# mengshanfeng/stencil-2

Hardware: AMD Instinct MI355X
Metric: Jacobi3D Gcells/s (512^3/GPU weak scaling; halo-exchange GB/s in extra) (higher is better)
Workload: dtype fp32

## Files before the change

### csrc/include/stencil/kernels/stencil_ops.hpp

```cpp
#pragma once
#include <algorithm>
#include <cstdint>
#include <vector>

#include "stencil/core/geometry.hpp"
#include "stencil/domain/local_domain.hpp"

namespace stencil {

enum class StencilKind : int {
  Jacobi = 0,
  Astaroth = 1,
};

struct Spheres {
  bool enabled = false;
  Dim3 hot, cold;
  int64_t radius = 0;
  static Spheres jacobi(const Rect3 &cReg) {
    Spheres s;
    s.enabled = true;
    s.hot = Dim3(cReg.lo.x + (cReg.hi.x - cReg.lo.x) / 3, (cReg.lo.y + cReg.hi.y) / 2, (cReg.lo.z + cReg.hi.z) / 2);
    s.cold = Dim3(cReg.lo.x + (cReg.hi.x - cReg.lo.x) * 2 / 3, (cReg.lo.y + cReg.hi.y) / 2, (cReg.lo.z + cReg.hi.z) / 2);
    s.radius = (cReg.hi.x - cReg.lo.x) / 10;
    return s;
  }
};

struct StencilTune {
  int variant = 2;
  static constexpr int kMfma = 8;
  int ty = 2;
  int zchunk = 0;
  int nw = 8;
  int x3sched = 1;
  int x3parts = 0;
  float x3sphw = 0.45f;
  float x2sphw = 0.15f;
  bool x3sphchunk = true;
  int x3left = 3;
  bool x2early = true;
  int x2row = 1;
  int x2sched = 1;
  int x2xfast = 0;
  int x2reserve = 8;
  int reserveCUs = 0;
  bool x2lockstep = true;
  bool zslabRow = true;
  bool xcdRemap = true;
  bool nontemporal = true;
  bool alternateZ = true;
  int wrap = 0;
  uint64_t *publish = nullptr;
  uint64_t *blockClock = nullptr;
  int publishDepth = 0;
};
bool stencil7x2_row_kernel_used(const LocalDomain &dom, int64_t qi, const Rect3 &region, const StencilTune &tune);
int stencil7x2_wrappable_axes(const LocalDomain &dom, int64_t qi, int x2row = 1);

struct ForwardTarget {
  Dim3 dir;
  const LocalDomain *dst;
  Dim3 offset;
};

class HaloForwarder {
public:
  HaloForwarder(const LocalDomain &src, int64_t qi, const std::vector<ForwardTarget> &targets);
  ~HaloForwarder();
  HaloForwarder(const HaloForwarder &) = delete;
  HaloForwarder &operator=(const HaloForwarder &) = delete;
  const int *wm() const { return wm_; }
  const int *wp() const { return wp_; }
  int num_targets() const { return n_; }
  uint32_t mask(int parity) const { return mask_[parity]; }
  int64_t delta(int parity, int k) const { return delta_[parity][k]; }
  bool has_rest() const { return hasRest_; }
  void forward_rest(int parity, hipStream_t stream) const;
  static bool supported(const LocalDomain &dom, int64_t qi);

private:
  int wm_[3] = {0, 0, 0}, wp_[3] = {0, 0, 0};
  int n_ = 0;
  int dev_ = -1;
  uint32_t mask_[2] = {0, 0};
  int64_t delta_[2][27] = {};
  CopyPlan rest_[2];
  bool hasRest_ = false;
};

struct X3PlanInfo {
  int parts = 0, blocks = 0, groups = 0, lockstepGroups = 0, rounds = 0;
// ... 46 lines not shown
      r.rounds = 2;
    }
  }
  return r;
}

inline int64_t slots_less_reserved(int64_t resident, int reserveCUs, int cus) {
  const int64_t perCU = std::max<int64_t>(1, resident / std::max(1, cus));
  return std::max<int64_t>(perCU, resident - perCU * std::min(reserveCUs, cus / 2));
}

enum class X2Form : int { Row = 0, Ragged2, Ragged3, Tail, Col2, Column };
inline bool x2_row_form(X2Form f) { return f <= X2Form::Tail; }
inline bool x2_row_width(int64_t nx) { return nx > 256 && nx <= 832; }
inline X2Form stencil7x2_form(int64_t elemSize, int64_t nx, int64_t x0, int wrap, int x2row, bool publishing,
                              int64_t bufferBytes) {
  if (!x2row) return X2Form::Column;
  const int64_t V = 16 / elemSize, cw = 128 * V;
  const bool onChunk = x0 % V == 0;
  if (elemSize == 4 && (wrap & 1) && onChunk && x2_row_width(nx) && bufferBytes < (int64_t(1) << 32) - 4096) {
    return nx == 512 ? X2Form::Row : nx < 512 ? X2Form::Ragged2 : nx <= 768 ? X2Form::Ragged3 : X2Form::Tail;
  }
  return !publishing && onChunk && nx % cw == 0 ? X2Form::Col2 : X2Form::Column;
}

struct X2SweepSchedule {
  int seg = 1, parts = 0, rounds = 1;
  int64_t blocks = 0;
  int zc = 1, gz = 1;
};
X2SweepSchedule stencil7x2_schedule(X2Form form, int64_t cols, int nz, int64_t resident, int64_t slots,
                                    const StencilTune &tune);
struct X2LaunchInfo {
  X2Form form = X2Form::Column;
  int wrapVariant = 0;
  int64_t cols = 0, slots = 0;
  int seg = 0, parts = 0, rounds = 1;
  int64_t blocks = 0;
  int zchunk = 0, gz = 0;
};
X2LaunchInfo stencil7x2_launch_info(const LocalDomain &dom, int64_t qi, const Rect3 &region, StencilKind kind,
                                    const Spheres &sph, const StencilTune &tune = StencilTune());

struct X3Schedule {
  int seg = 1, parts = 0;
  int64_t blocks = 0;
  int rounds = 1;
};
X3Schedule stencil7x3_schedule(bool xh, int64_t cols, int64_t nz, int64_t slots, const StencilTune &tune,
                               bool publishing);
struct X3LaunchInfo {
  bool supported = false;
  bool xh = false, ragged = false;
  int64_t cols = 0, slots = 0;
  int seg = 0, parts = 0;
  int64_t blocks = 0;
  int rounds = 0;
};
X3LaunchInfo stencil7x3_launch_info(const LocalDomain &dom, int64_t qi, const Rect3 &region, StencilKind kind,
                                    const Spheres &sph, const StencilTune &tune);

int stencil7_wrappable_axes(const LocalDomain &dom, int64_t qi);
bool stencil7_mfma_supported(const LocalDomain &dom, int64_t qi);
void stencil7_mfma_apply(const LocalDomain &dom, int64_t qi, const Rect3 &region, StencilKind kind, const Spheres &sph,
                         hipStream_t stream, const StencilTune &tune = StencilTune());
void stencil7_apply_regions(const LocalDomain &dom, int64_t qi, const std::vector<Rect3> &regions, StencilKind kind,
                            const Spheres &sph, hipStream_t stream, const StencilTune &tune = StencilTune());

struct StarWeights {
  int radius = 1;
  double center = 0;
  double w[3][2][3] = {};
};
bool stencil_star_supported(const LocalDomain &dom, int64_t qi, const StarWeights &w);
void stencil_star_apply(const LocalDomain &dom, int64_t qi, const Rect3 &region, const StarWeights &w,
                        hipStream_t stream, const StencilTune &tune = StencilTune());
struct StarLaunchInfo {
  int path = 0;
  int zchunk = 0;
  int zchunks = 0;
  int64_t blocks = 0;
};
StarLaunchInfo stencil_star_launch_info(const LocalDomain &dom, int64_t qi, const Rect3 &region, const StarWeights &w,
                                        const StencilTune &tune = StencilTune());

struct BoxWeights {
  double w[3][3][3] = {};
};
bool stencil_box_supported(const LocalDomain &dom, int64_t qi);
void stencil_box_apply(const LocalDomain &dom, int64_t qi, const Rect3 &region, const BoxWeights &w,
                       hipStream_t stream, const StencilTune &tune = StencilTune());
struct BoxLaunchInfo {
  int path = 0;
  int zchunk = 0;
  int zchunks = 0;
  int64_t blocks = 0;
};
BoxLaunchInfo stencil_box_launch_info(const LocalDomain &dom, int64_t qi, const Rect3 &region, const BoxWeights &w,
                                      const StencilTune &tune = StencilTune());

struct VarCoefWeights {
  double shift = 0;
  double h[3] = {0, 0, 0};
};
bool stencil_varcoef_supported(const LocalDomain &dom, int64_t qu, int64_t qk);
void stencil_varcoef_apply(const LocalDomain &dom, int64_t qu, int64_t qk, const Rect3 &region, const VarCoefWeights &w,
// ... 27 lines not shown
```

### csrc/python/bindings.cpp

```cpp
#include <pybind11/functional.h>
#include <pybind11/pybind11.h>
#include <pybind11/stl.h>

#include <cstring>

#include <cmath>
#include <limits>
#include <sstream>

#include "stencil/comm/proc_group.hpp"
#include "stencil/comm/ipc_event.hpp"
#include "stencil/comm/rccl_comm.hpp"
#include "stencil/domain/distributed_domain.hpp"
#include "stencil/kernels/copy.hpp"
#include "stencil/kernels/grid_transfer.hpp"
#include "stencil/kernels/stencil_ops.hpp"
#include "stencil/models/stencil_model.hpp"
#include "stencil/rt/build_info.hpp"
#include "stencil/rt/statistics.hpp"
#include "stencil/topo/gpu_topology.hpp"
#include "stencil/topo/partition.hpp"
#include "stencil/topo/placement.hpp"
#include "stencil/topo/qap.hpp"

// ... 1228 lines not shown
                        const std::vector<BoundaryConditions> &bcs) {
          const FillLaunchInfo r = boundary_fill_launch_info(dd.domains().at(di), dd.size(), fill_requests(qs, bcs, true));
          static const char *names[] = {"none", "host", "generic", "fast"};
          py::dict o;
          o["path"] = names[r.path + 1];
          o["boxes"] = r.boxes;
          o["blocks"] = r.blocks;
          o["launches"] = r.launches;
          return o;
        },
        py::arg("dd"), py::arg("domain"), py::arg("qs"), py::arg("bcs"));
  m.def("set_boundary_fill_nontemporal", &set_boundary_fill_nontemporal, py::arg("on"));
  py::class_<X3PlanInfo>(m, "X3PlanInfo")
      .def_readonly("parts", &X3PlanInfo::parts)
      .def_readonly("blocks", &X3PlanInfo::blocks)
      .def_readonly("groups", &X3PlanInfo::groups)
      .def_readonly("lockstep_groups", &X3PlanInfo::lockstepGroups)
      .def_readonly("rounds", &X3PlanInfo::rounds)
      .def_readonly("tabled", &X3PlanInfo::tabled)
      .def_readonly("steps", &X3PlanInfo::steps)
      .def_readonly("zb", &X3PlanInfo::zb)
      .def_readonly("l0", &X3PlanInfo::l0)
      .def_readonly("l1", &X3PlanInfo::l1)
      .def_readonly("odd", &X3PlanInfo::odd)
      .def_readonly("marches", &X3PlanInfo::marches);
  m.def(
      "stencil7x3_plan",
      [](py::handle size, bool jacobi, py::object tune, int slots) {
        return stencil7x3_plan(to_dim3(size), jacobi, tune.is_none() ? StencilTune() : tune.cast<StencilTune>(), slots);
      },
      py::arg("size"), py::arg("jacobi"), py::arg("tune") = py::none(), py::arg("slots") = 256);
  m.def(
      "stencil7x3_schedule",
      [](bool xh, int64_t cols, int64_t nz, int64_t slots, py::object tune, bool publishing) {
        const X3Schedule r = stencil7x3_schedule(xh, cols, nz, slots,
                                                 tune.is_none() ? StencilTune() : tune.cast<StencilTune>(), publishing);
        return py::make_tuple(r.seg, r.parts, r.blocks, r.rounds);
      },
      py::arg("xh"), py::arg("cols"), py::arg("nz"), py::arg("slots"), py::arg("tune") = py::none(),
      py::arg("publishing") = false,
      "launch schedule of a fused-triple sweep (no GPU): (seg, parts, blocks, rounds) for the XH form (xh, columns with "
      "x halos) or the whole-row form over cols (row group, column) pairs of nz planes on `slots` resident blocks; seg "
      "1 = balanced split, 2 = lockstep parts plus second segments, 3 = lockstep rounds (XH form, not publishing)");
  m.def(
      "stencil7x3_launch_info",
      [](DistributedDomain &dd, size_t di, int64_t q, StencilKind kind, bool spheres, const StencilTune &tune) {
        const Spheres s = spheres ? Spheres::jacobi(dd.get_compute_region()) : Spheres();
        const LocalDomain &d = dd.domains().at(di);
        const X3LaunchInfo r = stencil7x3_launch_info(d, q, d.get_compute_region(), kind, s, tune);
        py::dict o;
        o["supported"] = r.supported;
        o["form"] = !r.supported ? "none" : (r.xh ? "xh" : "wrap");
        o["ragged"] = r.ragged;
        o["cols"] = r.cols;
        o["slots"] = r.slots;
        o["seg"] = r.seg;
        o["parts"] = r.parts;
        o["blocks"] = r.blocks;
        o["rounds"] = r.rounds;
        return o;
      },
      py::arg("dd"), py::arg("domain"), py::arg("qi"), py::arg("kind"), py::arg("spheres"), py::arg("tune"));
  m.def(
      "x2_lockstep_schedule",
      [](int64_t slots, int64_t cols, int64_t nz) {
        const X2Schedule r = x2_lockstep_schedule(slots, cols, nz);
        return py::make_tuple(r.parts, r.blocks, r.rounds);
      },
      py::arg("slots"), py::arg("cols"), py::arg("nz"),
      "lockstep schedule of the whole-row / two-chunk-column fused pairs: (z parts per row group, blocks, rounds of "
      "whole columns); (0, 0, 1) = balanced split");
  static const char *x2FormNames[] = {"row", "ragged2", "ragged3", "tail", "col2", "column"};
  m.def(
      "stencil7x2_form",
      [](int64_t elemSize, int64_t nx, int64_t x0, int wrap, int x2row, bool publishing, int64_t bufferBytes) {
        return x2FormNames[int(stencil7x2_form(elemSize, nx, x0, wrap, x2row, publishing, bufferBytes))];
      },
      py::arg("elem_size"), py::arg("nx"), py::arg("x0") = 0, py::arg("wrap") = 1, py::arg("x2row") = 1,
      py::arg("publishing") = false, py::arg("buffer_bytes") = 0,
      "kernel form of a fused-pair sweep (no GPU): \"row\" (512-cell periodic rows), \"ragged2\" / \"ragged3\" (257-511 / "
      "513-768 cells), \"tail\" (769-832), \"col2\" (two-chunk columns), \"column\" (the one-chunk column kernel); x0 = "
      "the region's first x cell counted from the first interior cell");
  m.def(
      "stencil7x2_schedule",
      [](const std::string &form, int64_t cols, int nz, int64_t resident, int64_t slots, py::object tune) {
        int f = 0;
        while (f < 6 && form != x2FormNames[f]) ++f;
        STENCIL_REQUIRE(f < 6, "fused-pair form " << form);
        const X2SweepSchedule r = stencil7x2_schedule(X2Form(f), cols, nz, resident, slots,
                                                      tune.is_none() ? StencilTune() : tune.cast<StencilTune>());
        py::dict o;
        o["seg"] = r.seg;
        o["parts"] = r.parts;
        o["rounds"] = r.rounds;
        o["blocks"] = r.blocks;
        o["zchunk"] = r.zc;
        o["gz"] = r.gz;
        return o;
      },
      py::arg("form"), py::arg("cols"), py::arg("nz"), py::arg("resident"), py::arg("slots"),
      py::arg("tune") = py::none(),
      "block schedule of a fused-pair sweep (no GPU): seg 0 = fixed z chunks (zchunk planes, gz per column), 1 = "
      "balanced split, 2 = lockstep parts plus second segments, 3 = lockstep rounds");
  m.def("slots_less_reserved", &slots_less_reserved, py::arg("resident"), py::arg("reserve_cus"), py::arg("cus"),
        "resident blocks a launch may fill when it leaves reserve_cus of the device's cus CUs to another stream");
  m.def(
      "stencil7x2_launch_info",
      [](DistributedDomain &dd, size_t di, int64_t q, const Rect3 &region, StencilKind kind, bool spheres,
         const StencilTune &tune) {
        const Spheres s = spheres ? Spheres::jacobi(dd.get_compute_region()) : Spheres();
        const X2LaunchInfo r = stencil7x2_launch_info(dd.domains().at(di), q, region, kind, s, tune);
        py::dict o;
        o["form"] = x2FormNames[int(r.form)];
        o["wrap_variant"] = r.wrapVariant;
        o["cols"] = r.cols;
        o["slots"] = r.slots;
        o["seg"] = r.seg;
        o["parts"] = r.parts;
        o["rounds"] = r.rounds;
        o["blocks"] = r.blocks;
        o["zchunk"] = r.zchunk;
        o["gz"] = r.gz;
        return o;
      },
      py::arg("dd"), py::arg("domain"), py::arg("qi"), py::arg("region"), py::arg("kind"), py::arg("spheres"),
      py::arg("tune"));
  m.def("jacobi_spheres", [](const Rect3 &cReg) {
    Spheres s = Spheres::jacobi(cReg);
    return py::make_tuple(s.hot, s.cold, s.radius);
  });

  py::class_<StencilTune>(m, "StencilTune")
      .def(py::init<>())
      .def_readwrite("variant", &StencilTune::variant)
      .def_readwrite("ty", &StencilTune::ty)
      .def_readwrite("zchunk", &StencilTune::zchunk)
      .def_readwrite("xcd_remap", &StencilTune::xcdRemap)
      .def_readwrite("nontemporal", &StencilTune::nontemporal)
      .def_readwrite("alternate_z", &StencilTune::alternateZ)
      .def_readwrite("nw", &StencilTune::nw)
      .def_readwrite("x3sched", &StencilTune::x3sched)
      .def_readwrite("x2early", &StencilTune::x2early)
      .def_readwrite("x3parts", &StencilTune::x3parts)
      .def_readwrite("x3sphw", &StencilTune::x3sphw)
      .def_readwrite("x3sphchunk", &StencilTune::x3sphchunk)
      .def_readwrite("x3left", &StencilTune::x3left)
      .def_readwrite("x2sphw", &StencilTune::x2sphw)
      .def_property(
          "block_clock", [](const StencilTune &t) { return reinterpret_cast<uintptr_t>(t.blockClock); },
          [](StencilTune &t, uintptr_t p) { t.blockClock = reinterpret_cast<uint64_t *>(p); })
      .def_readwrite("x2row", &StencilTune::x2row)
      .def_readwrite("x2sched", &StencilTune::x2sched)
      .def_readwrite("x2reserve", &StencilTune::x2reserve)
      .def_readwrite("wrap", &StencilTune::wrap)
      .def_readwrite("x2lockstep", &StencilTune::x2lockstep)
      .def_readwrite("zslab_row", &StencilTune::zslabRow)
      .def_readwrite("x2xfast", &StencilTune::x2xfast);
  py::class_<StencilModelConfig>(m, "StencilModelConfig")
      .def(py::init<>())
      .def_readwrite("size", &StencilModelConfig::size)
      .def_readwrite("kind", &StencilModelConfig::kind)
      .def_readwrite("radius", &StencilModelConfig::radius)
      .def_readwrite("all_directions", &StencilModelConfig::allDirections)
      .def_readwrite("quantities", &StencilModelConfig::quantities)
      .def_readwrite("fp64", &StencilModelConfig::fp64)
      .def_readwrite("methods", &StencilModelConfig::methods)
      .def_readwrite("placement", &StencilModelConfig::placement)
      .def_readwrite("axis_cost", &StencilModelConfig::axisCost)
      .def_readwrite("partition", &StencilModelConfig::partition)
      .def_readwrite("gpus", &StencilModelConfig::gpus)
      .def_readwrite("overlap", &StencilModelConfig::overlap)
      .def_readwrite("auto_overlap", &StencilModelConfig::autoOverlap)
      .def_readwrite("use_graph", &StencilModelConfig::useGraph)
      .def_readwrite("forward", &StencilModelConfig::forward)
      .def_readwrite("temporal", &StencilModelConfig::temporal)
      .def_readwrite("wrap_self", &StencilModelConfig::wrapSelf)
      .def_readwrite("x_halo_align", &StencilModelConfig::xHaloAlign)
      .def_readwrite("shared_halo_line", &StencilModelConfig::sharedHaloLine)
      .def_readwrite("interior_align", &StencilModelConfig::interiorAlign)
      .def_readwrite("row_pad_lines", &StencilModelConfig::rowPadLines)
      .def_readwrite("wrap_axes_mask", &StencilModelConfig::wrapAxesMask)
      .def_readwrite("local_interior", &StencilModelConfig::localInterior)
      .def_readwrite("overlap_mode", &StencilModelConfig::overlapMode)
      .def_readwrite("transport", &StencilModelConfig::transport)
      .def_readwrite("self_test", &StencilModelConfig::selfTest)
      .def_property(
          "backend", [](const StencilModelConfig &c) { return c.backend; },
          [](StencilModelConfig &c, Backend b) {
            c.backend = b;
            c.setBackend = true;
          })
      .def_readwrite("tune", &StencilModelConfig::tune)
      .def_readwrite("astaroth_period", &StencilModelConfig::astarothPeriod);
  py::class_<StencilModel, std::shared_ptr<StencilModel>>(m, "StencilModel")
      .def(py::init([](const StencilModelConfig &c, std::shared_ptr<comm::ProcGroup> pg) {
             py::gil_scoped_release r;
             return std::make_shared<StencilModel>(c, pg);
           }),
// ... 34 lines not shown
```

### csrc/src/kernels/stencil7x3.hip

```cpp
#include <hip/hip_runtime.h>

#include <algorithm>
#include <map>
#include <mutex>
#include <utility>
#include <vector>
#include <cmath>
#include <cstring>

#include "stencil/kernels/stencil_ops.hpp"
#include "stencil/rt/hip_check.hpp"
#include "stencil_common.hpp"
#include "stencil_wave.hpp"

namespace stencil {

struct X3Seg {
  uint32_t s, e, s2, e2;
  bool odd;
  bool odd2;
};
template <typename T>
__host__ __device__ __forceinline__ X3Seg x3_segments(const StencilArgs<T> &a, const ZPartBounds &B, uint32_t lb,
                                                      uint32_t nb, uint32_t ncols, uint32_t gy, uint32_t nzt) {
// ... 407 lines not shown
            for (int h = 0; h < H; ++h) {
              U1b[h] = U1c[h];
              U1c[h] = U1a[h];
              U2b[h] = U2c[h];
              U2c[h] = U2a[h];
            }
            if constexpr (EDGE) {
              U1Eb = U1Ec;
              U1Ec = U1Ea;
            }
            ++t;
            return true;
          };
          using I0 = std::integral_constant<int, 0>;
          using I1 = std::integral_constant<int, 1>;
          using I2 = std::integral_constant<int, 2>;
          using I3 = std::integral_constant<int, 3>;
          using L1 = std::integral_constant<int, (RM < 1 ? RM : 1)>;
          using L2 = std::integral_constant<int, (RM < 2 ? RM : 2)>;
          using LR = std::integral_constant<int, RM>;
          step(I0{}, L1{});
          step(I1{}, L1{});
          step(I2{}, L2{});
          step(I3{}, L2{});
          while (step(I0{}, LR{}) && step(I1{}, LR{}) && step(I2{}, LR{}) && step(I3{}, LR{})) {
          }
        };
        if (down)
          march(std::true_type{});
        else
          march(std::false_type{});
      }
    }
  };
  const unsigned long long clk0 = a.clk ? wall_clock64() : 0;
  const int role = (w >= 3 && w < NW - 3) ? 3 : ((w >= 2 && w < NW - 2) ? 2 : ((w >= 1 && w < NW - 1) ? 1 : 0));
  if (role == 3)
    body(std::integral_constant<int, 3>{});
  else if (role == 2)
    body(std::integral_constant<int, 2>{});
  else if (role == 1)
    body(std::integral_constant<int, 1>{});
  else
    body(std::integral_constant<int, 4>{});
  if (a.clk) {
    __syncthreads();
    if (lane == 0 && w == 0) {
      a.clk[2 * lb] = clk0;
      a.clk[2 * lb + 1] = wall_clock64();
    }
  }
}

template <int KIND, bool PUB, bool NT>
__global__ __launch_bounds__(64 * 12, 3) __attribute__((amdgpu_waves_per_eu(3, 3))) void
stencil7x3_wrap_kernel(StencilArgs<float> a, ZPartBounds zbounds) {
  constexpr int NW = 12;
  using T = float;
  using NV = nf4;
  constexpr int V = 4, H = 2;
  constexpr int CS = 64 * V;
  constexpr int LS = V;
  constexpr int YO = NW - 6;
  constexpr int NC = 4;
  __shared__ NV cs[2][NW][H][64];
  __shared__ NV us[2][NW][H][64];
  __shared__ NV vs[2][NW][H][64];

  const uint32_t nb = gridDim.x;
  const uint32_t lb = a.remap ? xcd_remap(blockIdx.x, nb) : blockIdx.x;
  const int lane = threadIdx.x;
  const int w = __builtin_amdgcn_readfirstlane(int(threadIdx.y));
  const uint32_t nzt = uint32_t(a.hiz - a.loz);
  const X3Seg sg = x3_segments(a, zbounds, lb, nb, uint32_t(a.gy), uint32_t(a.gy), nzt);
  const bool lane0 = lane == 0, lane63 = lane == 63;
  const int wA = w > 0 ? w - 1 : 0, wB = w < NW - 1 ? w + 1 : NW - 1;
  const int xb = a.lox + lane * LS;
  const int zwn = a.wn[2], zwlo = a.wlo[2], zwhi = a.wlo[2] + a.wn[2];
  const __amdgpu_buffer_rsrc_t srcRsrc =
      __builtin_amdgcn_make_buffer_rsrc(const_cast<float *>(a.src), 0, -1, 0x00020000);
  auto zcl = [&](int zz) {
    zz += zz < zwlo ? zwn : 0;
    zz -= zz >= zwhi ? zwn : 0;
    return zz < 0 ? 0 : (zz > a.rawZm1 ? a.rawZm1 : zz);
  };
  auto body = [&](auto roleTag) {
    constexpr int R = decltype(roleTag)::value;
    bool odd = sg.odd;
    const bool pubOrder = PUB;
    for (int pp = 0; pp < 2; ++pp) {
      const int pass = pubOrder ? 1 - pp : pp;
      uint32_t s = pass == 0 ? sg.s : sg.s2;
      const uint32_t e = pass == 0 ? sg.e : sg.e2;
      if (pass == 1 && !pubOrder) odd = sg.odd2;
      while (s < e) {
        const uint32_t by = s / nzt;
        const int zo = int(s - by * nzt);
        const int nzs = int(min(nzt - uint32_t(zo), e - s));
        s += uint32_t(nzs);
        const int zs = a.loz + zo;
        const int ze = zs + nzs;
        bool down = pass == 0 && sg.odd;
        if (!pubOrder) {
          down = odd != (a.flip != 0);
          odd = !odd;
        }
        const int yblk = a.loy + YO * int(by);
        const int y = yblk - 3 + w;
        if (yblk >= a.hiy) continue;
        const bool outRow = R == 3 && y < a.hiy;
        int yw = y < a.wlo[1] ? y + a.wn[1] : (y >= a.wlo[1] + a.wn[1] ? y - a.wn[1] : y);
        yw = yw < 0 ? 0 : (yw > a.rawYm1 ? a.rawYm1 : yw);
        const uint32_t rowoff = uint32_t((yw * int64_t(a.px) + xb) * int64_t(sizeof(T)));
        const uint32_t outoff = uint32_t((y * int64_t(a.px) + xb) * int64_t(sizeof(T)));

        const int yh = a.r1sq - (y - a.hy) * (y - a.hy), yc = a.r1sq - (y - a.cy) * (y - a.cy);
        struct RowSph {
          int Dh, Dc;
          bool hit;
        };
        auto row_sph = [&](int P) -> RowSph {
          RowSph r{0, 0, false};
          if (KIND == 0) {
            r.Dh = yh - (P - a.hz) * (P - a.hz);
            r.Dc = yc - (P - a.cz) * (P - a.cz);
            r.hit = max(r.Dh, r.Dc) > 0;
          }
          return r;
        };
        auto sphere_row = [&](const RowSph &rs, NV(&o)[H]) {
          if (KIND == 0 && rs.hit) {
            const int Dh = rs.Dh, Dc = rs.Dc;
#pragma unroll
            for (int h = 0; h < H; ++h)
#pragma unroll
              for (int k = 0; k < V; ++k) {
                const int x = xb + h * CS + k;
                const bool hot = (x - a.hx) * (x - a.hx) < Dh;
                const bool cold = (x - a.cx) * (x - a.cx) < Dc;
                o[h][k] = hot ? T(1) : (cold ? T(0) : o[h][k]);
              }
          }
        };
        auto row_update = [&](const NV(&cm)[H], const NV(&up)[H], const NV(&dn)[H], const NV(&zp)[H], const NV(&zm)[H],
                              NV(&o)[H]) -> T {
          static_assert(H == 2, "two chunks per lane");
          const T r30 = rot_prev(cm[0][V - 1]), r31 = rot_prev(cm[1][V - 1]);
          const T l00 = rot_next(cm[0][0]), l01 = rot_next(cm[1][0]);
          NV s6[H];
#pragma unroll
          for (int h = 0; h < H; ++h) {
            const T left = h == 0 ? (lane0 ? r31 : r30) : (lane0 ? r30 : r31);
            const T right = h == 0 ? (lane63 ? l01 : l00) : (lane63 ? l00 : l01);
            NV vpx, vmx;
#pragma unroll
            for (int k = 0; k < V; ++k) {
              vpx[k] = k < V - 1 ? cm[h][k + 1] : right;
              vmx[k] = k > 0 ? cm[h][k - 1] : left;
            }
            s6[h] = sum6v<T, KIND>(vpx, vmx, dn[h], up[h], zp[h], zm[h]);
          }
          float m = 1.0f;
#pragma unroll
          for (int h = 0; h < H; ++h) o[h] = div6v_fast<NV, V>(s6[h], m);
          if (__builtin_expect(m < 0x1p-100f, 0)) {
#pragma unroll
            for (int h = 0; h < H; ++h) div6v_fix<NV, V>(s6[h], o[h]);
          }
          return T(1);
        };

        auto march = [&](auto downTag) {
          constexpr bool DOWN = decltype(downTag)::value;
          constexpr int dz = DOWN ? -1 : 1;
          const int z0 = DOWN ? ze - 1 : zs;
          NV C[NC][H];
          NV U1a[H], U1b[H], U1c[H];
          NV U2a[H], U2b[H], U2c[H];
          auto load_row = [&](int zz, int k) {
            const uint32_t po = uint32_t(zcl(zz)) * uint32_t(a.pxy) * uint32_t(sizeof(T));
#pragma unroll
            for (int h = 0; h < H; ++h)
              C[k][h] = __builtin_bit_cast(
                  NV, __builtin_amdgcn_raw_buffer_load_b128(srcRsrc, rowoff + uint32_t(h * CS * int(sizeof(T))), po, 0));
          };
          {
            const int zw = z0 - 3 * dz;
#pragma unroll
            for (int k = 0; k < NC - 1; ++k) load_row(zw + k * dz, k);
#pragma unroll
// ... 44 lines not shown
                sphere_row(row_sph(z), o);
              }
            };
            levels();
            if constexpr (LV >= 3) {
              char *dp = outRow ? reinterpret_cast<char *>(a.dst + int64_t(z) * a.pxy) + outoff
                                : a.sink + lane * LS * int(sizeof(T));
#pragma unroll
              for (int h = 0; h < H; ++h) {
                NV *q = reinterpret_cast<NV *>(dp + h * CS * int(sizeof(T)));
                if constexpr (NT)
                  __builtin_nontemporal_store(o[h], q);
                else
                  *q = o[h];
              }
            }
            const int nbuf = buf ^ 1;
            if constexpr (LV < 1)
#pragma unroll
              for (int h = 0; h < H; ++h) cs[nbuf][w][h][lane] = C[s2][h];
            const bool pubStep = PUB && t >= 0 && (z < a.pubLo || z >= a.pubHi);
            if (pubStep) asm volatile("s_waitcnt vmcnt(0)" ::: "memory");
            __syncthreads();
            if (pubStep && lane == 0 && w == 0) {
              __builtin_amdgcn_fence(__ATOMIC_RELEASE, "");
              const unsigned long long cells =
                  (unsigned long long)(min(YO, a.hiy - yblk)) * (unsigned long long)(a.hix - a.lox);
              __hip_atomic_fetch_add(a.pub, cells, __ATOMIC_RELAXED, __HIP_MEMORY_SCOPE_SYSTEM);
            }
#pragma unroll
            for (int h = 0; h < H; ++h) {
              U1b[h] = U1c[h];
              U1c[h] = U1a[h];
              U2b[h] = U2c[h];
              U2c[h] = U2a[h];
            }
            ++t;
            return true;
          };
          using I0 = std::integral_constant<int, 0>;
          using I1 = std::integral_constant<int, 1>;
          using I2 = std::integral_constant<int, 2>;
          using I3 = std::integral_constant<int, 3>;
          using L1 = std::integral_constant<int, (R < 1 ? R : 1)>;
          using L2 = std::integral_constant<int, (R < 2 ? R : 2)>;
          using LR = std::integral_constant<int, R>;
          step(I0{}, L1{});
          step(I1{}, L1{});
          step(I2{}, L2{});
          step(I3{}, L2{});
          while (step(I0{}, LR{}) && step(I1{}, LR{}) && step(I2{}, LR{}) && step(I3{}, LR{})) {
          }
        };
        if (down)
          march(std::true_type{});
        else
          march(std::false_type{});
      }
    }
  };
  const unsigned long long clk0 = a.clk ? wall_clock64() : 0;
  const int role = (w >= 3 && w < NW - 3) ? 3 : ((w >= 2 && w < NW - 2) ? 2 : ((w >= 1 && w < NW - 1) ? 1 : 0));
  if (role == 3)
    body(std::integral_constant<int, 3>{});
  else if (role == 2)
    body(std::integral_constant<int, 2>{});
  else if (role == 1)
    body(std::integral_constant<int, 1>{});
  else
    body(std::integral_constant<int, 0>{});
  if (a.clk) {
    __syncthreads();
    if (lane == 0 && w == 0) {
      a.clk[2 * lb] = clk0;
      a.clk[2 * lb + 1] = wall_clock64();
    }
  }
}

template <typename T, int KIND> static const void *x3_wrap_kernel_ptr(bool nt) {
  if constexpr (std::is_same<T, float>::value)
    return nt ? (const void *)stencil7x3_wrap_kernel<KIND, false, true>
              : (const void *)stencil7x3_wrap_kernel<KIND, false, false>;
  else
    return nullptr;
}
template <typename T, int KIND> using X3XhKernel = void (*)(StencilArgs<T>, ZPartBounds);
template <typename T, int KIND, bool BIG, bool PUB> static X3XhKernel<T, KIND> x3_xh_kernel_ptr(bool rag) {
  return rag ? stencil7x3_xh_kernel<T, KIND, BIG, PUB, true> : stencil7x3_xh_kernel<T, KIND, BIG, PUB, false>;
}
template <typename T, int KIND> static X3XhKernel<T, KIND> x3_xh_kernel_ptr(bool big, bool pub, bool rag) {
  return big ? (pub ? x3_xh_kernel_ptr<T, KIND, true, true>(rag) : x3_xh_kernel_ptr<T, KIND, true, false>(rag))
             : (pub ? x3_xh_kernel_ptr<T, KIND, false, true>(rag) : x3_xh_kernel_ptr<T, KIND, false, false>(rag));
}

static std::map<int, char *> gX3Sinks;
static std::mutex gX3SinkMu;
static char *x3_sink(int dev, bool create) {
  std::lock_guard<std::mutex> lk(gX3SinkMu);
  char *&p = gX3Sinks[dev];
  if (!p && create) {
    int cur = 0;
    HIP_CHECK(hipGetDevice(&cur));
    HIP_CHECK(hipSetDevice(dev));
    HIP_CHECK(hipMalloc(reinterpret_cast<void **>(&p), 4096));
    HIP_CHECK(hipSetDevice(cur));
  }
  return p;
}

int64_t stencil7x3_column_cells(int64_t elemSize) { return 2 * 64 * (16 / elemSize); }

bool stencil7x3_supported(const LocalDomain &dom, int64_t qi, const Rect3 &region, const StencilTune &tune) {
  if (dom.backend() != Backend::Device) return false;
  const int64_t es = dom.elem_size(qi);
  const bool f32 = dom.dtype(qi) == DType::F32 || (dom.dtype(qi) == DType::Bytes && es == 4);
  const bool f64 = dom.dtype(qi) == DType::F64 || (dom.dtype(qi) == DType::Bytes && es == 8);
  if (!f32 && !f64) return false;
  const Radius &rad = dom.radius();
  const Dim3 n = dom.size();
  const int wrapm = tune.wrap & 7;
  if (wrapm & 1) {
    if (!f32 || n.x != 512 || !(stencil7x2_wrappable_axes(dom, qi, 1) & 1)) return false;
  } else {
    const int64_t cw = stencil7x3_column_cells(es);
    if (rad.x(-1) < 3 || rad.x(1) < 3 || n.x < 3 || n.x % cw > cw - 3) return false;
  }
  if (!(wrapm & 2) && (rad.y(-1) < 3 || rad.y(1) < 3)) return false;
  if (!(wrapm & 4) && (rad.z(-1) < 3 || rad.z(1) < 3)) return false;
  for (int i = 0; i < 27; ++i) {
    const Dim3 d = dir_from_index(i);
    const int nzc = (d.x != 0) + (d.y != 0) + (d.z != 0);
    const bool halo = !((d.x != 0 && (wrapm & 1)) || (d.y != 0 && (wrapm & 2)) || (d.z != 0 && (wrapm & 4)));
    if (nzc >= 2 && halo && rad.dir(d) < 1) return false;
  }
  const Rect3 cr = dom.get_compute_region();
// ... 63 lines not shown
static X3Plan x3_plan(const StencilArgs<T> &a, bool jac, int64_t cols, int64_t slots, uint32_t blocks,
                      const StencilTune &tune) {
  constexpr int NW = 12, YO = NW - 6;
  constexpr double kUnsync = 1.2;
  const int64_t nz = a.hiz - a.loz;
  const float w = jac ? tune.x3sphw : 0.f;
  auto plan = [&](int P, int64_t nbP, ZPartBounds &b) -> double {
    b = ZPartBounds{};
    const int64_t cm = nbP / P;
    if (jac) sphere_part_bounds(b, a, std::min<int64_t>(cm, a.gy), P, NW, YO, 3, w);
    const int mode = tune.x3left;
    ZPartBounds bg = b, bl = b;
    const double tg = mode == 1 || mode == 3
                          ? balance_leftover(bg, a, nbP, cm, P, cols, a.gy, NW, YO, 3, w, 4, mode == 3 ? kUnsync : 1.0)
                          : -1;
    const double tl = mode == 2 || mode == 3 ? lockstep_leftover(bl, a, nbP, cm, P, cols, a.gy, NW, YO, 3, w, 4, 16) : -1;
    if (tl >= 0 && (tg < 0 || tl <= tg)) {
      b = bl;
      return tl;
    }
    if (tg >= 0) {
      b = bg;
      return tg;
    }
    const std::vector<double> mc = lockstep_part_costs(b, a, cm, P, a.gy, NW, YO, 3, w, 4);
    const double left = cols > cm ? double((cols - cm) * nz) * kUnsync / double(nbP) + 4 : 0;
    return *std::max_element(mc.begin(), mc.end()) + left;
  };
  X3Plan pl{a.zparts, blocks, ZPartBounds{}, 0};
  if (tune.x3sched == 1 && tune.x3parts <= 0 && tune.x3left != 0) {
    double best = -1;
    const bool sph = jac && a.r1sq > 0 && w > 0;
    for (int P = 2; P <= (sph ? kZPartMaxParts : 8); ++P) {
      const int64_t cm = std::min<int64_t>(cols, slots / P);
      if (cm < 1 || nz / P < 16) continue;
      ZPartBounds b;
      const double t = plan(P, P * cm, b);
      if (best < 0 || t < best - 1e-9) {
        best = t;
        pl = X3Plan{P, uint32_t(P * cm), b, t};
      }
    }
  } else {
    pl.steps = plan(a.zparts, int64_t(blocks), pl.b);
  }
  return pl;
}

template <typename T> struct X3Launch {
  StencilArgs<T> a;
  ZPartBounds zb;
  uint32_t blocks;
  bool big, rag;
  int64_t cols, slots;
};
template <typename T, int KIND, bool XH>
static X3Launch<T> x3_prepare(const LocalDomain &dom, int64_t qi, const Rect3 &region, const Spheres &sph,
                              const StencilTune &tune) {
  constexpr int NW = 12, YO = NW - 6;
  X3Launch<T> L{};
  StencilArgs<T> &a = L.a;
  a = make_args<T>(dom, qi, region, KIND == 0 ? StencilKind::Jacobi : StencilKind::Astaroth, sph);
  a.flip = tune.alternateZ ? (dom.parity() & 1) : 0;
  a.nt = tune.nontemporal ? 1 : 0;
  a.wrapm = tune.wrap & 7;
  if (!(a.wrapm & 2)) a.wn[1] = 0;
  if (!(a.wrapm & 4)) a.wn[2] = 0;
  a.x0 = a.lox;
  a.remap = tune.xcdRemap ? 1 : 0;
  a.sphchunk = tune.x3sphchunk ? 1 : 0;
  a.sphr = int(sph.radius);
  const int nx = a.hix - a.lox, ny = a.hiy - a.loy, nz = a.hiz - a.loz;
  const int cw = int(stencil7x3_column_cells(int64_t(sizeof(T))));
  a.gx = XH ? (nx + cw - 1) / cw : 1;
  a.xr = XH ? nx - (a.gx - 1) * cw : nx;
  const bool rag = XH && a.xr < cw;
  a.gy = (ny + YO - 1) / YO;
  const bool big = dom.buffer_bytes(qi) >= (int64_t(1) << 32) - 4096;
  const void *kern =
      XH ? (const void *)x3_xh_kernel_ptr<T, KIND>(big, false, rag) : x3_wrap_kernel_ptr<T, KIND>(a.nt != 0);
  const int64_t cols = int64_t(a.gx) * a.gy;
  const int64_t resident = resident_blocks(kern, 64 * NW, 1);
  const int64_t slots = launch_slots(resident, tune.reserveCUs, dom.gpu());
  if (tune.publish) {
    a.pub = reinterpret_cast<unsigned long long *>(tune.publish);
    a.pubLo = a.loz + tune.publishDepth;
    a.pubHi = a.hiz - tune.publishDepth;
    a.flip = 0;
  }
  const X3Schedule ls = stencil7x3_schedule(XH, cols, nz, slots, tune, tune.publish != nullptr);
  a.seg = ls.seg;
  uint32_t blocks = uint32_t(ls.blocks);
  if (ls.seg != 1) {
    a.zparts = ls.parts;
    a.zrounds = ls.rounds;
  }
  ZPartBounds &zb = L.zb;
  if (a.seg == 2) {
    static std::map<std::vector<int64_t>, X3Plan> cache;
    static std::mutex mu;
    int32_t wbits = 0;
    std::memcpy(&wbits, &tune.x3sphw, sizeof(wbits));
    const std::vector<int64_t> key{KIND, a.loy,  a.hiy, a.loz, a.hiz,          a.hy,        a.cy,
                                   a.hz, a.cz,   a.r1sq, int64_t(blocks), a.zparts, cols, a.gy,
                                   wbits, tune.x3left, tune.x3sched, tune.x3parts, slots};
    std::lock_guard<std::mutex> lk(mu);
    auto it = cache.find(key);
    if (it == cache.end()) it = cache.emplace(key, x3_plan(a, KIND == 0, cols, slots, blocks, tune)).first;
    a.zparts = it->second.P;
    blocks = it->second.blocks;
    zb = it->second.b;
  }
  a.sink = x3_sink(dom.gpu(), false);
  a.clk = reinterpret_cast<unsigned long long *>(tune.blockClock);
  L.blocks = blocks;
  L.big = big;
  L.rag = rag;
  L.cols = cols;
  L.slots = slots;
  return L;
}

template <typename T, int KIND, bool XH>
static void apply_x3_t(const LocalDomain &dom, int64_t qi, const Rect3 &region, const Spheres &sph, hipStream_t stream,
                       const StencilTune &tune) {
  constexpr int NW = 12;
  const X3Launch<T> L = x3_prepare<T, KIND, XH>(dom, qi, region, sph, tune);
  const StencilArgs<T> &a = L.a;
  const ZPartBounds &zb = L.zb;
  const uint32_t blocks = L.blocks;
  dom.set_device();
  STENCIL_REQUIRE(a.sink, "stencil7x3: no store sink on device " << dom.gpu() << " (stencil7x3_supported first)");
  if constexpr (XH || !std::is_same<T, float>::value) {
    const X3XhKernel<T, KIND> k = x3_xh_kernel_ptr<T, KIND>(L.big, a.pub != nullptr, L.rag);
    hipLaunchKernelGGL(k, dim3(blocks), dim3(64, NW), 0, stream, a, zb);
  } else {
    if (a.pub)
      hipLaunchKernelGGL((stencil7x3_wrap_kernel<KIND, true, false>), dim3(blocks), dim3(64, NW), 0, stream, a, zb);
    else if (a.nt)
      hipLaunchKernelGGL((stencil7x3_wrap_kernel<KIND, false, true>), dim3(blocks), dim3(64, NW), 0, stream, a, zb);
    else
      hipLaunchKernelGGL((stencil7x3_wrap_kernel<KIND, false, false>), dim3(blocks), dim3(64, NW), 0, stream, a, zb);
  }
  HIP_CHECK(hipGetLastError());
}

static std::vector<int> x3_marches(const StencilArgs<float> &a, const ZPartBounds &zb, uint32_t nb) {
  constexpr int YO = 6;
  std::vector<int> out;
  const uint32_t nzt = uint32_t(a.hiz - a.loz);
  for (uint32_t lb = 0; lb < nb; ++lb) {
    const X3Seg sg = x3_segments(a, zb, lb, nb, uint32_t(a.gy), uint32_t(a.gy), nzt);
    bool odd = sg.odd;
    for (int pass = 0; pass < 2; ++pass) {
      uint32_t s = pass == 0 ? sg.s : sg.s2;
      const uint32_t e = pass == 0 ? sg.e : sg.e2;
      if (pass == 1) odd = sg.odd2;
      while (s < e) {
        const uint32_t by = s / nzt;
        const int zo = int(s - by * nzt);
        const int nzs = int(std::min(nzt - uint32_t(zo), e - s));
        s += uint32_t(nzs);
        const bool down = odd != (a.flip != 0);
        odd = !odd;
        if (a.loy + YO * int(by) >= a.hiy) continue;
        out.insert(out.end(), {int(lb), int(by), a.loz + zo, nzs, int(down)});
      }
    }
  }
  return out;
}

X3PlanInfo stencil7x3_plan(const Dim3 &size, bool jacobi, const StencilTune &tune, int slots) {
  constexpr int YO = 6;
  StencilArgs<float> a{};
  a.hix = int(size.x);
  a.hiy = int(size.y);
  a.hiz = int(size.z);
  if (jacobi) {
    const Spheres s = Spheres::jacobi(Rect3(Dim3(0, 0, 0), size));
    a.hx = int(s.hot.x);
    a.hy = int(s.hot.y);
    a.hz = int(s.hot.z);
    a.cx = int(s.cold.x);
    a.cy = int(s.cold.y);
    a.cz = int(s.cold.z);
    a.r1sq = int((s.radius + 1) * (s.radius + 1));
  }
  a.gx = 1;
  a.gy = int((size.y + YO - 1) / YO);
  const int64_t cols = a.gy, nz = size.z;
  X3PlanInfo r;
  r.groups = int(cols);
  const X3Schedule ls = stencil7x3_schedule(false, cols, nz, slots, tune, tune.publish != nullptr);
  r.parts = ls.parts;
  r.blocks = ls.seg == 1 ? 0 : int(ls.blocks);
  r.rounds = ls.rounds;
  a.seg = ls.seg;
  if (ls.seg != 2) {
    r.marches = x3_marches(a, ZPartBounds{}, uint32_t(ls.blocks));
    return r;
  }
  a.zparts = ls.parts;
  const X3Plan pl = x3_plan(a, jacobi, cols, slots, uint32_t(ls.blocks), tune);
  a.zparts = pl.P;
  r.marches = x3_marches(a, pl.b, pl.blocks);
  r.parts = pl.P;
  r.blocks = int(pl.blocks);
  r.lockstepGroups = int(pl.blocks) / pl.P;
  r.steps = pl.steps;
  r.tabled = pl.b.lon != 0;
  if (pl.b.on)
    for (int g = 0; g < std::min<int>(r.lockstepGroups, kZPartMaxCols); ++g)
      for (int q = 0; q + 1 < pl.P; ++q) r.zb.push_back(pl.b.zb[g][q]);
  if (r.tabled)
    for (uint32_t lb = 0; lb < pl.blocks; ++lb) {
      r.l0.push_back(pl.b.l0[lb]);
      r.l1.push_back(pl.b.l1[lb]);
      r.odd.push_back(int((pl.b.ldir[lb / 32] >> (lb % 32)) & 1));
    }
  return r;
}

bool stencil7x3_apply(const LocalDomain &dom, int64_t qi, const Rect3 &region, StencilKind kind, const Spheres &sph,
                      hipStream_t stream, const StencilTune &tune) {
  if (!stencil7x3_supported(dom, qi, region, tune)) return false;
  const bool jac = kind == StencilKind::Jacobi, xh = !(tune.wrap & 1);
  if (dom.elem_size(qi) == 8) {
    jac ? apply_x3_t<double, 0, true>(dom, qi, region, sph, stream, tune)
        : apply_x3_t<double, 1, true>(dom, qi, region, sph, stream, tune);
  } else if (xh) {
    jac ? apply_x3_t<float, 0, true>(dom, qi, region, sph, stream, tune)
        : apply_x3_t<float, 1, true>(dom, qi, region, sph, stream, tune);
  } else {
    jac ? apply_x3_t<float, 0, false>(dom, qi, region, sph, stream, tune)
        : apply_x3_t<float, 1, false>(dom, qi, region, sph, stream, tune);
  }
  return true;
}

template <typename T, int KIND, bool XH>
static X3LaunchInfo x3_launch_info_t(const LocalDomain &dom, int64_t qi, const Rect3 &region, const Spheres &sph,
                                     const StencilTune &tune) {
  const X3Launch<T> L = x3_prepare<T, KIND, XH>(dom, qi, region, sph, tune);
  X3LaunchInfo r;
  r.supported = true;
  r.xh = XH;
  r.ragged = L.rag;
  r.cols = L.cols;
  r.slots = L.slots;
  r.seg = L.a.seg;
  r.parts = L.a.seg == 1 ? 0 : L.a.zparts;
  r.blocks = int64_t(L.blocks);
  r.rounds = L.a.seg == 3 ? L.a.zrounds : 1;
  return r;
}

X3LaunchInfo stencil7x3_launch_info(const LocalDomain &dom, int64_t qi, const Rect3 &region, StencilKind kind,
                                    const Spheres &sph, const StencilTune &tune) {
  if (!stencil7x3_supported(dom, qi, region, tune)) return X3LaunchInfo();
  const bool jac = kind == StencilKind::Jacobi, xh = !(tune.wrap & 1);
  if (dom.elem_size(qi) == 8)
    return jac ? x3_launch_info_t<double, 0, true>(dom, qi, region, sph, tune)
               : x3_launch_info_t<double, 1, true>(dom, qi, region, sph, tune);
  if (xh)
    return jac ? x3_launch_info_t<float, 0, true>(dom, qi, region, sph, tune)
               : x3_launch_info_t<float, 1, true>(dom, qi, region, sph, tune);
  return jac ? x3_launch_info_t<float, 0, false>(dom, qi, region, sph, tune)
             : x3_launch_info_t<float, 1, false>(dom, qi, region, sph, tune);
}

}
```

Before: 1942.

## Stage fused-triple wrap march rows via buffer-load-to-LDS DMA ring

Adds a DMA variant of the wrap-form fused triple stencil kernel. Input z-rows are loaded directly into an LDS ring with buffer_load_lds, and intermediate sweep levels are exchanged through LDS, with explicit vmcnt/lgkmcnt waits and barriers per step. The aim is to remove register staging of global loads and overlap prefetch of rows several planes ahead with compute. It adds a sizeable shared-memory array that may reduce residency, and it is enabled by a new x3dma tune flag that defaults on but only applies to the non-publishing wrap form.

New measurement: 1856. 4.4% lower.

```diff
diff --git a/csrc/include/stencil/kernels/stencil_ops.hpp b/csrc/include/stencil/kernels/stencil_ops.hpp
--- a/csrc/include/stencil/kernels/stencil_ops.hpp
+++ b/csrc/include/stencil/kernels/stencil_ops.hpp
@@ -38,6 +38,7 @@
   float x3sphw = 0.45f;
   float x2sphw = 0.15f;
   bool x3sphchunk = true;
+  bool x3dma = true;
   int x3left = 3;
   bool x2early = true;
   int x2row = 1;
@@ -190,6 +191,7 @@
 struct X3LaunchInfo {
   bool supported = false;
   bool xh = false, ragged = false;
+  bool dma = false;
   int64_t cols = 0, slots = 0;
   int seg = 0, parts = 0;
   int64_t blocks = 0;
diff --git a/csrc/python/bindings.cpp b/csrc/python/bindings.cpp
--- a/csrc/python/bindings.cpp
+++ b/csrc/python/bindings.cpp
@@ -1304,6 +1304,7 @@
         o["supported"] = r.supported;
         o["form"] = !r.supported ? "none" : (r.xh ? "xh" : "wrap");
         o["ragged"] = r.ragged;
+        o["dma"] = r.dma;
         o["cols"] = r.cols;
         o["slots"] = r.slots;
         o["seg"] = r.seg;
@@ -1396,6 +1397,7 @@
       .def_readwrite("x3parts", &StencilTune::x3parts)
       .def_readwrite("x3sphw", &StencilTune::x3sphw)
       .def_readwrite("x3sphchunk", &StencilTune::x3sphchunk)
+      .def_readwrite("x3dma", &StencilTune::x3dma)
       .def_readwrite("x3left", &StencilTune::x3left)
       .def_readwrite("x2sphw", &StencilTune::x2sphw)
       .def_property(
diff --git a/csrc/src/kernels/stencil7x3.hip b/csrc/src/kernels/stencil7x3.hip
--- a/csrc/src/kernels/stencil7x3.hip
+++ b/csrc/src/kernels/stencil7x3.hip
@@ -483,9 +483,10 @@
   }
 }
 
-template <int KIND, bool PUB, bool NT>
+template <int KIND, bool PUB, bool NT, bool DMA = false>
 __global__ __launch_bounds__(64 * 12, 3) __attribute__((amdgpu_waves_per_eu(3, 3))) void
 stencil7x3_wrap_kernel(StencilArgs<float> a, ZPartBounds zbounds) {
+  static_assert(!(PUB && DMA), "the publishing instances keep the register-staged march");
   constexpr int NW = 12;
   using T = float;
   using NV = nf4;
@@ -497,6 +498,8 @@
   __shared__ NV cs[2][NW][H][64];
   __shared__ NV us[2][NW][H][64];
   __shared__ NV vs[2][NW][H][64];
+  constexpr int XU1 = 3 * NW, XU2 = XU1 + 2 * (NW - 2), XROWS = XU2 + 2 * (NW - 4);
+  __shared__ NV xl[XROWS * H * 64];
 
   const uint32_t nb = gridDim.x;
   const uint32_t lb = a.remap ? xcd_remap(blockIdx.x, nb) : blockIdx.x;
@@ -562,11 +565,13 @@
         auto sphere_row = [&](const RowSph &rs, NV(&o)[H]) {
           if (KIND == 0 && rs.hit) {
             const int Dh = rs.Dh, Dc = rs.Dc;
+            int xo = xb;
+            if constexpr (DMA) asm volatile("" : "+v"(xo));
 #pragma unroll
             for (int h = 0; h < H; ++h)
 #pragma unroll
               for (int k = 0; k < V; ++k) {
-                const int x = xb + h * CS + k;
+                const int x = xo + h * CS + k;
                 const bool hot = (x - a.hx) * (x - a.hx) < Dh;
                 const bool cold = (x - a.cx) * (x - a.cx) < Dc;
                 o[h][k] = hot ? T(1) : (cold ? T(0) : o[h][k]);
@@ -717,10 +722,157 @@
           while (step(I0{}, LR{}) && step(I1{}, LR{}) && step(I2{}, LR{}) && step(I3{}, LR{})) {
           }
         };
-        if (down)
-          march(std::true_type{});
-        else
-          march(std::false_type{});
+
+        auto march_dma = [&](auto downTag) {
+          constexpr bool DOWN = decltype(downTag)::value;
+          constexpr int dz = DOWN ? -1 : 1;
+          const int z0 = DOWN ? ze - 1 : zs;
+          NV W[3][H];
+          NV NA[H], NB[H];
+          NV U1a[H], U1b[H], U1c[H];
+          NV U2a[H], U2b[H], U2c[H];
+          typedef __attribute__((address_space(3))) NV LNV;
+          auto rowbase = [&](int row) -> uint32_t {
+            uint32_t b = uint32_t(reinterpret_cast<uintptr_t>(&xl[row * H * 64 + lane]));
+            asm("" : "+v"(b));
+            return b;
+          };
+          auto u1row = [&](int r) { return XU1 + min(max(r, 1), NW - 2) - 1; };
+          auto u2row = [&](int r) { return XU2 + min(max(r, 2), NW - 3) - 2; };
+          const uint32_t rW = rowbase(w), rA = rowbase(wA), rB = rowbase(wB);
+          const uint32_t uW = rowbase(u1row(w)), uA = rowbase(u1row(wA)), uB = rowbase(u1row(wB));
+          const uint32_t vW = rowbase(u2row(w)), vA = rowbase(u2row(wA)), vB = rowbase(u2row(wB));
+          auto at = [&](uint32_t base, int off) -> LNV & { return *reinterpret_cast<LNV *>(base + uint32_t(off)); };
+          auto ring = [&](uint32_t base, int slot, int h) -> LNV & { return at(base, (slot * NW * H + h) * 1024); };
+          auto u1s = [&](uint32_t base, int b, int h) -> LNV & { return at(base, (b * (NW - 2) * H + h) * 1024); };
+          auto u2s = [&](uint32_t base, int b, int h) -> LNV & { return at(base, (b * (NW - 4) * H + h) * 1024); };
+          auto dma_row = [&](int zz, int slot) {
+            const uint32_t po = uint32_t(zcl(zz)) * uint32_t(a.pxy) * uint32_t(sizeof(T));
+#pragma unroll
+            for (int h = 0; h < H; ++h)
+              __builtin_amdgcn_raw_ptr_buffer_load_lds(
+                  srcRsrc, (__attribute__((address_space(3))) void *)&xl[((slot * NW + w) * H + h) * 64], 16,
+                  rowoff + uint32_t(h * CS * int(sizeof(T))), po, 0, 0);
+          };
+          {
+            dma_row(z0 - 3 * dz, 0);
+            dma_row(z0 - 2 * dz, 1);
+            dma_row(z0 - dz, 2);
+            asm volatile("s_waitcnt vmcnt(0)" ::: "memory");
+            __builtin_amdgcn_s_barrier();
+#pragma unroll
+            for (int h = 0; h < H; ++h) {
+              W[0][h] = ring(rW, 0, h);
+              W[1][h] = W[2][h] = NA[h] = NB[h] = W[0][h];
+              U1a[h] = U1b[h] = U1c[h] = U2a[h] = U2b[h] = U2c[h] = W[0][h];
+            }
+            asm volatile("s_waitcnt lgkmcnt(0)" ::: "memory");
+          }
+          int t = -5;
+          auto step = [&](auto phase, auto lvTag, auto psTag) -> bool {
+            constexpr int k = decltype(phase)::value;
+            constexpr int LV = decltype(lvTag)::value;
+            constexpr bool PS = decltype(psTag)::value;
+            constexpr int s0 = (k + 1) % 3, s1 = (k + 2) % 3, s2 = k % 3, sn = (k + 2) % 3;
+            constexpr int buf = k & 1;
+            if (t >= nzs) return false;
+            const int z = z0 + t * dz;
+            dma_row(z + 5 * dz, sn);
+            __builtin_amdgcn_sched_barrier(0);
+            NV o[H];
+            if constexpr (R >= 1) {
+              NV A2[H], B2[H], A3[H], B3[H];
+#pragma unroll
+              for (int h = 0; h < H; ++h) W[s2][h] = ring(rW, s2, h);
+              if constexpr (LV >= 1) {
+                (void)row_update(W[s1], NA, NB, DOWN ? W[s0] : W[s2], DOWN ? W[s2] : W[s0], U1a);
+                sphere_row(row_sph(z + 2 * dz), U1a);
+#pragma unroll
+                for (int h = 0; h < H; ++h) u1s(uW, buf ^ 1, h) = U1a[h];
+              }
+#pragma unroll
+              for (int h = 0; h < H; ++h) {
+                NA[h] = ring(rA, s2, h);
+                NB[h] = ring(rB, s2, h);
+              }
+              if constexpr (LV >= 2) {
+#pragma unroll
+                for (int h = 0; h < H; ++h) {
+                  A2[h] = u1s(uA, buf, h);
+                  B2[h] = u1s(uB, buf, h);
+                }
+                (void)row_update(U1c, A2, B2, DOWN ? U1b : U1a, DOWN ? U1a : U1b, U2a);
+                sphere_row(row_sph(z + dz), U2a);
+#pragma unroll
+                for (int h = 0; h < H; ++h) u2s(vW, buf ^ 1, h) = U2a[h];
+              }
+              if constexpr (LV >= 3) {
+#pragma unroll
+                for (int h = 0; h < H; ++h) {
+                  A3[h] = u2s(vA, buf, h);
+                  B3[h] = u2s(vB, buf, h);
+                }
+                (void)row_update(U2c, A3, B3, DOWN ? U2b : U2a, DOWN ? U2a : U2b, o);
+                sphere_row(row_sph(z), o);
+                char *dp = outRow ? reinterpret_cast<char *>(a.dst + int64_t(z) * a.pxy) + outoff
+                                  : a.sink + lane * LS * int(sizeof(T));
+#pragma unroll
+                for (int h = 0; h < H; ++h) {
+                  NV *q = reinterpret_cast<NV *>(dp + h * CS * int(sizeof(T)));
+                  if constexpr (NT)
+                    __builtin_nontemporal_store(o[h], q);
+                  else
+                    *q = o[h];
+                }
+              }
+            }
+            constexpr int N = 2 + (LV >= 3 ? 2 : 0) + (PS ? 2 : 0);
+            asm volatile("s_waitcnt vmcnt(%0)\n\ts_waitcnt lgkmcnt(0)" ::"n"(N) : "memory");
+            __builtin_amdgcn_s_barrier();
+#pragma unroll
+            for (int h = 0; h < H; ++h) {
+              U1b[h] = U1c[h];
+              U1c[h] = U1a[h];
+              U2b[h] = U2c[h];
+              U2c[h] = U2a[h];
+            }
+            ++t;
+            return true;
+          };
+          using I0 = std::integral_constant<int, 0>;
+          using I1 = std::integral_constant<int, 1>;
+          using I2 = std::integral_constant<int, 2>;
+          using I3 = std::integral_constant<int, 3>;
+          using I4 = std::integral_constant<int, 4>;
+          using I5 = std::integral_constant<int, 5>;
+          using L0 = std::integral_constant<int, 0>;
+          using L1 = std::integral_constant<int, (R < 1 ? R : 1)>;
+          using L2 = std::integral_constant<int, (R < 2 ? R : 2)>;
+          using LR = std::integral_constant<int, R>;
+          using PN = std::false_type;
+          using PY = std::integral_constant<bool, R == 3>;
+          step(I1{}, L0{}, PN{});
+          step(I2{}, L1{}, PN{});
+          step(I3{}, L1{}, PN{});
+          step(I4{}, L2{}, PN{});
+          step(I5{}, L2{}, PN{});
+          step(I0{}, LR{}, PN{});
+          while (step(I1{}, LR{}, PY{}) && step(I2{}, LR{}, PY{}) && step(I3{}, LR{}, PY{}) && step(I4{}, LR{}, PY{}) &&
+                 step(I5{}, LR{}, PY{}) && step(I0{}, LR{}, PY{})) {
+          }
+          asm volatile("s_waitcnt vmcnt(0)" ::: "memory");
+        };
+        if constexpr (DMA) {
+          if (down)
+            march_dma(std::true_type{});
+          else
+            march_dma(std::false_type{});
+        } else {
+          if (down)
+            march(std::true_type{});
+          else
+            march(std::false_type{});
+        }
       }
     }
   };
@@ -743,10 +895,15 @@
   }
 }
 
-template <typename T, int KIND> static const void *x3_wrap_kernel_ptr(bool nt) {
+using X3WrapKernel = void (*)(StencilArgs<float>, ZPartBounds);
+template <int KIND> static X3WrapKernel x3_wrap_kernel(bool pub, bool nt, bool dma) {
+  if (pub) return stencil7x3_wrap_kernel<KIND, true, false>;
+  if (dma) return nt ? stencil7x3_wrap_kernel<KIND, false, true, true> : stencil7x3_wrap_kernel<KIND, false, false, true>;
+  return nt ? stencil7x3_wrap_kernel<KIND, false, true> : stencil7x3_wrap_kernel<KIND, false, false>;
+}
+template <typename T, int KIND> static const void *x3_wrap_kernel_ptr(bool nt, bool dma) {
   if constexpr (std::is_same<T, float>::value)
-    return nt ? (const void *)stencil7x3_wrap_kernel<KIND, false, true>
-              : (const void *)stencil7x3_wrap_kernel<KIND, false, false>;
+    return (const void *)x3_wrap_kernel<KIND>(false, nt, dma);
   else
     return nullptr;
 }
@@ -916,6 +1073,7 @@
   ZPartBounds zb;
   uint32_t blocks;
   bool big, rag;
+  bool dma;
   int64_t cols, slots;
 };
 template <typename T, int KIND, bool XH>
@@ -942,7 +1100,7 @@
   a.gy = (ny + YO - 1) / YO;
   const bool big = dom.buffer_bytes(qi) >= (int64_t(1) << 32) - 4096;
   const void *kern =
-      XH ? (const void *)x3_xh_kernel_ptr<T, KIND>(big, false, rag) : x3_wrap_kernel_ptr<T, KIND>(a.nt != 0);
+      XH ? (const void *)x3_xh_kernel_ptr<T, KIND>(big, false, rag) : x3_wrap_kernel_ptr<T, KIND>(a.nt != 0, tune.x3dma);
   const int64_t cols = int64_t(a.gx) * a.gy;
   const int64_t resident = resident_blocks(kern, 64 * NW, 1);
   const int64_t slots = launch_slots(resident, tune.reserveCUs, dom.gpu());
@@ -980,6 +1138,7 @@
   L.blocks = blocks;
   L.big = big;
   L.rag = rag;
+  L.dma = !XH && tune.x3dma && !tune.publish;
   L.cols = cols;
   L.slots = slots;
   return L;
@@ -999,12 +1158,8 @@
     const X3XhKernel<T, KIND> k = x3_xh_kernel_ptr<T, KIND>(L.big, a.pub != nullptr, L.rag);
     hipLaunchKernelGGL(k, dim3(blocks), dim3(64, NW), 0, stream, a, zb);
   } else {
-    if (a.pub)
-      hipLaunchKernelGGL((stencil7x3_wrap_kernel<KIND, true, false>), dim3(blocks), dim3(64, NW), 0, stream, a, zb);
-    else if (a.nt)
-      hipLaunchKernelGGL((stencil7x3_wrap_kernel<KIND, false, true>), dim3(blocks), dim3(64, NW), 0, stream, a, zb);
-    else
-      hipLaunchKernelGGL((stencil7x3_wrap_kernel<KIND, false, false>), dim3(blocks), dim3(64, NW), 0, stream, a, zb);
+    hipLaunchKernelGGL(x3_wrap_kernel<KIND>(a.pub != nullptr, a.nt != 0, L.dma), dim3(blocks), dim3(64, NW), 0, stream,
+                       a, zb);
   }
   HIP_CHECK(hipGetLastError());
 }
@@ -1111,6 +1266,7 @@
   r.supported = true;
   r.xh = XH;
   r.ragged = L.rag;
+  r.dma = L.dma;
   r.cols = L.cols;
   r.slots = L.slots;
   r.seg = L.a.seg;
```
